# Enigmatisms/NeRF

Measured on AMD Instinct MI355X. Metric: rays/s (64+128 samples), 800x800, higher is better.
Workload: dtype bf16

## Files before the change

nerf_amd/csrc/sample_kernels.hip:

```cpp
#include "device_common.h"
#include "host_common.h"
#include "../../include/nerf_amd.h"
#include "launchers.h"

extern __shared__ __attribute__((aligned(16))) char smem[];

namespace {

constexpr int WAVES_PER_BLOCK = 4;

DEVINL int wave_in_block() { return (int)(threadIdx.x >> 6); }

constexpr int ENC_TILE = 64;
static inline size_t enc_lds_bytes(int L) { return (size_t)ENC_TILE * (6 * L + 6) * 4; }
template <bool IPE, class Moments>
DEVINL void encode_tile(float (*mom)[6], float* stage, int64_t base, int64_t total, int L, float* __restrict__ feat, Moments&& moments) {
    const int width = 6 * L, pairs_per = 3 * L;
    const int nsamp = (int)(total - base < ENC_TILE ? total - base : ENC_TILE);
    if ((int)threadIdx.x < nsamp) moments((int)threadIdx.x, base + threadIdx.x);
    __syncthreads();
    const int n_pairs = nsamp * pairs_per;
    for (int p = threadIdx.x; p < n_pairs; p += blockDim.x) {
        const int sl = p / pairs_per, rem = p - sl * pairs_per;
        const int l = rem / 3, c = rem - 3 * l;
// ... 305 lines not shown
            const int64_t k = cell / wp, r = cell - k * wp;
            const int64_t wr = r / ww;
            const int64_t row = y0 + wr, col = x0 + (r - wr * ww);
            const int64_t v = view_ids != nullptr ? view_ids[k] : k;
            float* q = ray_s[threadIdx.x];
            if (v >= 0 && v < V) {
                pixel_camera_ray((int)col, (int)row, cameras + v * NERF_AMD_CAMERA_ROW, poses + v * 12, q);
                const float* px = images + ((v * 3) * (int64_t)H + row) * W + col;
#pragma unroll
                for (int c = 0; c < 6; ++c) rays[n * 6 + c] = q[c];
#pragma unroll
                for (int c = 0; c < 3; ++c) rgb[n * 3 + c] = px[(int64_t)c * H * W];
                if (index != nullptr) index[n] = (v * H + row) * W + col;
            } else {
                const float nan = __builtin_nanf("");
#pragma unroll
                for (int c = 0; c < 6; ++c) { q[c] = nan; rays[n * 6 + c] = nan; }
#pragma unroll
                for (int c = 0; c < 3; ++c) rgb[n * 3 + c] = nan;
                if (index != nullptr) index[n] = -1;
            }
        }
        __syncthreads();
        if (lengths == nullptr) continue;
        sampler_samples(n0, N, C, seed, near, res, ray_s, lengths, pts);
    }
}

__global__ void length2pts_kernel(const float* __restrict__ rays, const float* __restrict__ z, int64_t N, int S,
                                  float* __restrict__ out) {
    const int64_t total = N * S * 6;
    for (int64_t i = blockIdx.x * (int64_t)blockDim.x + threadIdx.x; i < total; i += (int64_t)gridDim.x * blockDim.x) {
        const int64_t ns = i / 6;
        const int k = (int)(i - ns * 6);
        const int64_t n = ns / S;
        const float* r = rays + n * 6;
        out[i] = (k < 3) ? (r[k] + r[3 + k] * z[ns]) : r[k];
    }
}

__global__ __launch_bounds__(256) void sigma_to_weights_kernel(const float* __restrict__ sigma, const float* __restrict__ z,
                                                              const float* __restrict__ dirs, int64_t N, int S, int act,
                                                              float* __restrict__ w) {
    for (int64_t n = blockIdx.x * (int64_t)WAVES_PER_BLOCK + wave_in_block(); n < N; n += (int64_t)gridDim.x * WAVES_PER_BLOCK) {
        float nrm = 1.0f;
        const bool scale = dirs != nullptr;
        if (scale) nrm = norm3(dirs[n * 3], dirs[n * 3 + 1], dirs[n * 3 + 2]);
        const float* sg = sigma + n * S;
        const float* zz = z + n * S;
        float* wo = w + n * S;
        wave_sigma_to_weights(S, act, [&](int s) { return sg[s]; },
                              [&](int s) { return scale ? zz[s] * nrm : zz[s]; },
                              [&](int s, float wv, float) { wo[s] = wv; });
    }
}

DEVINL float max_blur_at(const float* w, int s, int S, float alpha) {
    const float c = w[s];
    const float front = (s == 0) ? c : fmaxf(w[s - 1], c);
    const float rear = (s == S - 1) ? c : fmaxf(c, w[s + 1]);
    return 0.5f * (front + rear) + alpha;
}
__global__ void max_blur_kernel(const float* __restrict__ w, int64_t N, int S, float alpha, float* __restrict__ out) {
    const int64_t total = N * S;
    for (int64_t i = blockIdx.x * (int64_t)blockDim.x + threadIdx.x; i < total; i += (int64_t)gridDim.x * blockDim.x) {
        const int s = (int)(i % S);
        out[i] = max_blur_at(w + (i - s), s, S, alpha);
    }
}

DEVINL void lds_wave_sync() {
    __builtin_amdgcn_fence(__ATOMIC_RELEASE, "workgroup");
    __builtin_amdgcn_wave_barrier();
    __builtin_amdgcn_fence(__ATOMIC_ACQUIRE, "workgroup");
}

#ifndef SORT_NB_DEF
#define SORT_NB_DEF 256
#define SORT_CAP_DEF 6
#endif
constexpr int SORT_NB = SORT_NB_DEF, SORT_CAP = SORT_CAP_DEF, SORT_PER_LANE = SORT_NB / 64;
constexpr int SORT_LDS_FLOATS = 2 * SORT_NB + SORT_NB * SORT_CAP / 2;

template <class UF>
DEVINL void wave_inverse_sample(const float* pw, const float* bins, int nw, float* cdf, float* samp, int* bel, int* sortbuf,
                                UF&& uf, int K, int sort, float* __restrict__ z_out,
                                int64_t* __restrict__ below_out, int64_t* __restrict__ above_out) {
    const int lane = lane_id();
    const int nb = nw + 1;
    float* part8 = reinterpret_cast<float*>(sortbuf);
    const int nv = nw >> 3;
    if (lane < 8) {
        const int n4 = nv >> 2;
        float a0 = 0.0f, a1 = 0.0f, a2 = 0.0f, a3 = 0.0f;
        for (int i = 0; i < n4; ++i) {
            a0 += pw[32 * i + lane] + 1e-5f;
            a1 += pw[32 * i + 8 + lane] + 1e-5f;
            a2 += pw[32 * i + 16 + lane] + 1e-5f;
            a3 += pw[32 * i + 24 + lane] + 1e-5f;
        }
        for (int v = 4 * n4; v < nv; ++v) a0 += pw[8 * v + lane] + 1e-5f;
        a0 += a1; a0 += a2; a0 += a3;
        part8[lane] = a0;
    }
    lds_wave_sync();
    float total = 0.0f;
    if (nv > 0) {
        for (int j = 8 * nv; j < nw; ++j) total += pw[j] + 1e-5f;
#pragma unroll
        for (int c = 0; c < 8; ++c) total += part8[c];
    } else {
        float a1 = 0.0f, a2 = 0.0f, a3 = 0.0f;
        if (nw >= 4) { total += pw[0] + 1e-5f; a1 += pw[1] + 1e-5f; a2 += pw[2] + 1e-5f; a3 += pw[3] + 1e-5f; }
        for (int j = nw & ~3; j < nw; ++j) total += pw[j] + 1e-5f;
        total += a1; total += a2; total += a3;
    }
    double carry = 0.0;
    if (lane == 0) cdf[0] = 0.0f;
    for (int base = 0; base < nw; base += 64) {
        const int j = base + lane;
        double p = 0.0;
        if (j < nw) p = (double)((pw[j] + 1e-5f) / total);
        const double incl = wave_incl_scan_add(p);
        if (j < nw) cdf[1 + j] = (float)(carry + incl);
        carry += wave_last(incl);
    }
    lds_wave_sync();
    const int halvings = 32 - __builtin_clz((unsigned)nb);
    for (int k0 = 0, i0 = 0; k0 < K; k0 += 192, i0 += 3) {
        float uu[3]; int lo[3], hi[3];
#pragma unroll
        for (int q = 0; q < 3; ++q) {
            const int k = k0 + 64 * q + lane;
            uu[q] = (k < K) ? uf(i0 + q, k) : 0.0f;
            lo[q] = 0; hi[q] = (k < K) ? nb : 0;
        }
        for (int it = 0; it < halvings; ++it) {
#pragma unroll
            for (int q = 0; q < 3; ++q) {
                const int mid = (lo[q] + hi[q]) >> 1;
                const bool open_ = lo[q] < hi[q];
                const float c = cdf[open_ ? mid : 0];
                if (open_) { if (c <= uu[q]) lo[q] = mid + 1; else hi[q] = mid; }
            }
        }
#pragma unroll
        for (int q = 0; q < 3; ++q) {
            const int k = k0 + 64 * q + lane;
            if (k >= K) continue;
            const int below = lo[q] - 1 > 0 ? lo[q] - 1 : 0;
            const int above = lo[q] < nb - 1 ? lo[q] : nb - 1;
            const float c0 = cdf[below], c1 = cdf[above];
            float denom = c1 - c0;
            if (denom < 1e-5f) denom = 1.0f;
            const float t = (uu[q] - c0) / denom;
            const float b0 = bins[below], b1 = bins[above];
            const float v = b0 + t * (b1 - b0);
            if (sort) { samp[k] = v; bel[k] = below; }
            else {
                z_out[k] = v;
                if (below_out) below_out[k] = below;
                if (above_out) above_out[k] = above;
            }
        }
    }
    if (!sort) return;
    lds_wave_sync();
    int* cnt = sortbuf;
    int* pre = sortbuf + SORT_NB;
    unsigned short* mem = reinterpret_cast<unsigned short*>(sortbuf + 2 * SORT_NB);
    for (int b = lane; b < SORT_NB; b += 64) cnt[b] = 0;
    lds_wave_sync();
    int overflow = 0, risky = -1;
    for (int j = lane; j + 1 < nb; j += 64) {
        const float b0 = bins[j], b1 = bins[j + 1];
        overflow |= (b1 < b0) ? 1 : 0;
        const bool exact = b0 >= 0.0f ? (b1 <= 2.0f * b0 || b0 == 0.0f) : (b1 <= 0.0f && b0 >= 2.0f * b1);
        if (!exact) risky = j;
    }
    if (__any(risky >= 0)) {
        risky = wave_max_i(risky);
        for (int k = lane; k < K; k += 64) {
            const int bl = bel[k];
            if (bl <= risky) overflow |= (samp[k] > bins[bl + 1]) ? 1 : 0;
        }
    }
    for (int k = lane, i = 0; k < K; k += 64, ++i) {
        int b = (int)(uf(i, k) * (float)SORT_NB);
        b = b < 0 ? 0 : (b > SORT_NB - 1 ? SORT_NB - 1 : b);
        const int pos = atomicAdd(&cnt[b], 1);
        if (pos < SORT_CAP) mem[b * SORT_CAP + pos] = (unsigned short)k; else overflow = 1;
    }
    lds_wave_sync();
    if (__any(overflow)) {
        for (int k = lane; k < K; k += 64) {
            const float v = samp[k];
            int rank = 0;
            for (int j = 0; j < K; ++j) {
                const float o = samp[j];
                rank += (o < v || (o == v && j < k)) ? 1 : 0;
            }
            z_out[rank] = v;
            if (below_out) below_out[rank] = bel[k];
        }
        return;
    }
    {
        int c[SORT_PER_LANE], tot = 0;
#pragma unroll
        for (int i = 0; i < SORT_PER_LANE; ++i) { c[i] = cnt[lane * SORT_PER_LANE + i]; tot += c[i]; }
        int run = wave_incl_scan_add(tot) - tot;
#pragma unroll
        for (int i = 0; i < SORT_PER_LANE; ++i) { pre[lane * SORT_PER_LANE + i] = run; run += c[i]; }
    }
    lds_wave_sync();
    for (int k0 = 0, i0 = 0; k0 < K; k0 += 192, i0 += 3) {
        float v[3]; int rank[3], cntb[3], bb[3];
#pragma unroll
        for (int q = 0; q < 3; ++q) {
            const int k = k0 + 64 * q + lane;
            const bool ok = k < K;
            int b = ok ? (int)(uf(i0 + q, k) * (float)SORT_NB) : 0;
            b = b < 0 ? 0 : (b > SORT_NB - 1 ? SORT_NB - 1 : b);
            bb[q] = b;
            v[q] = samp[ok ? k : 0];
            rank[q] = pre[b];
            cntb[q] = ok ? cnt[b] : 0;
        }
        int most = cntb[0] > cntb[1] ? cntb[0] : cntb[1];
        most = most > cntb[2] ? most : cntb[2];
        const int trips = wave_max_i(most);
        for (int p = 0; p < trips; ++p) {
#pragma unroll
            for (int q = 0; q < 3; ++q) {
                const int k = k0 + 64 * q + lane;
                const bool live = p < cntb[q];
                const int jx = mem[bb[q] * SORT_CAP + p];
                const float o = samp[live ? jx : 0];
                rank[q] += (live && (o < v[q] || (o == v[q] && jx < k))) ? 1 : 0;
            }
        }
#pragma unroll
        for (int q = 0; q < 3; ++q) {
            const int k = k0 + 64 * q + lane;
            if (k >= K) continue;
            z_out[rank[q]] = v[q];
            if (below_out) below_out[rank[q]] = bel[k];
        }
    }
}

template <class P> struct ResampleRowsAt { P pw, bins, cdf, samp, bel, sortbuf, zl, wraw, tail; };
typedef ResampleRowsAt<float*> ResampleRows;
template <class P> static inline __host__ __device__ ResampleRowsAt<P> resample_rows(P base, int C, int K) {
    ResampleRowsAt<P> r;
    r.pw = base; r.bins = r.pw + C; r.cdf = r.bins + C; r.samp = r.cdf + C; r.bel = r.samp + K; r.sortbuf = r.bel + K;
    r.zl = r.sortbuf + SORT_LDS_FLOATS; r.wraw = r.zl + C; r.tail = r.wraw + C;
    return r;
}
static inline __host__ __device__ size_t inv_lds_floats(int C, int K) { return resample_rows<size_t>(0, C, K).zl; }
static inline __host__ __device__ size_t rs_lds_floats(int C, int K) { return resample_rows<size_t>(0, C, K).tail; }
static inline __host__ __device__ size_t warped_lds_floats(int C, int K) { return rs_lds_floats(C, K) + (size_t)2 * K; }
static inline __host__ __device__ size_t rsw_lds_floats(int C, int K, bool warped) { return rs_lds_floats(C, K) + (size_t)(warped ? 2 : 1) * K; }
DEVINL ResampleRows wave_resample_rows(size_t wave_floats, int C, int K) {
    return resample_rows(reinterpret_cast<float*>(smem) + wave_in_block() * wave_floats, C, K);
}
template <class UF>
DEVINL void wave_inverse_sample(const ResampleRows& r, int nw, UF&& uf, int K, int sort, float* __restrict__ z_out, int64_t* __restrict__ below_out,
                                int64_t* __restrict__ above_out) {
    wave_inverse_sample(r.pw, r.bins, nw, r.cdf, r.samp, reinterpret_cast<int*>(r.bel), reinterpret_cast<int*>(r.sortbuf), uf, K, sort, z_out, below_out,
                        above_out);
}

DEVINL void wave_blur_pdf(const float* wraw, int C, float alpha, float* pw, float* w_prop) {
    for (int j = lane_id(); j < C; j += 64) {
        const float wb = max_blur_at(wraw, j, C, alpha);
        if (j >= 1 && j <= C - 2) pw[j - 1] = wb;
        if (w_prop) w_prop[j] = wb;
    }
}
DEVINL void wave_midpoints(const float* x, int C, float* bins) {
    for (int j = lane_id(); j < C - 1; j += 64) bins[j] = 0.5f * (x[j + 1] + x[j]);
}

__global__ __launch_bounds__(256) void inverse_sample_kernel(const float* __restrict__ w, const float* __restrict__ z,
                                                            const float* __restrict__ u, int64_t N, int C, int K, int sort,
                                                            int mode, float* __restrict__ z_out, int64_t* __restrict__ below,
                                                            int64_t* __restrict__ above) {
    const ResampleRows r = wave_resample_rows(inv_lds_floats(C, K), C, K);
    float* const pw = r.pw; float* const bins = r.bins;
    const int lane = lane_id();
    const int nw = mode == 0 ? C - 2 : C - 1;
    const int wstride = mode == 0 ? C : C - 1;
    for (int64_t n = blockIdx.x * (int64_t)WAVES_PER_BLOCK + wave_in_block(); n < N; n += (int64_t)gridDim.x * WAVES_PER_BLOCK) {
        lds_wave_sync();
        if (mode == 0) {
            for (int j = lane; j < nw; j += 64) pw[j] = w[n * wstride + 1 + j];
            wave_midpoints(z + n * C, C, bins);
        } else {
            for (int j = lane; j < nw; j += 64) pw[j] = w[n * wstride + j];
            for (int j = lane; j < nw + 1; j += 64) bins[j] = z[n * C + j];
        }
        lds_wave_sync();
        const float* un = u + n * K;
        wave_inverse_sample(r, nw, [&](int, int k) { return un[k]; }, K, sort, z_out + n * K, below ? below + n * K : nullptr,
                            above ? above + n * K : nullptr);
    }
}

struct ResampleArgs {
    const float* density; const float* z; const float* z_base; const float* u_strat; float z_jitter;
    const float* dirs; int dirs_stride; const float* u_inv; int64_t N; int C; int K; int softplus; float alpha;
    float* z_fine; int64_t* below; float* w_prop; float* z_coarse;
    uint64_t rng_seed; int64_t rng_ray_offset;
};

#ifndef RS_BLOCKS_PER_CU
#define RS_BLOCKS_PER_CU 5
#endif
__global__ __launch_bounds__(256) __attribute__((amdgpu_waves_per_eu(RS_BLOCKS_PER_CU, RS_BLOCKS_PER_CU))) void resample_kernel(ResampleArgs a) {
    const int C = a.C, K = a.K;
    const ResampleRows rows = wave_resample_rows(rs_lds_floats(C, K), C, K);
    float* const zl = rows.zl; float* const wraw = rows.wraw;
    const int lane = lane_id();
    struct RayIn { float dx, dy, dz, zv0, zv1, dens0, dens1, u0, u1, u2; };
    const bool fits = C <= 128 && K <= 192;
    auto load_in = [&](int64_t n) -> RayIn {
        RayIn r;
        const float* dd = a.dirs + n * a.dirs_stride;
        r.dx = dd[0]; r.dy = dd[1]; r.dz = dd[2];
        Philox4 blk = {{0u, 0u, 0u, 0u}};
        const bool draw = !a.u_inv || (!a.z && !a.u_strat);
        if (draw) blk = philox_ray_block(a.rng_seed, n + a.rng_ray_offset, lane);
        auto depth_of = [&](int j, bool first) {
            if (a.z) return a.z[n * C + j];
            const float uu = a.u_strat ? a.u_strat[n * C + j] : (first ? u01_from_bits(blk.w[0]) : philox_u_strat(a.rng_seed, n + a.rng_ray_offset, j));
            return a.z_base[j] + uu * a.z_jitter;
        };
        r.zv0 = r.zv1 = r.dens0 = r.dens1 = 0.0f;
        if (lane < C) { r.zv0 = depth_of(lane, true); r.dens0 = a.density[n * C + lane]; }
        if (lane + 64 < C) { r.zv1 = depth_of(lane + 64, false); r.dens1 = a.density[n * C + lane + 64]; }
        if (a.u_inv) {
            const float* un = a.u_inv + n * K;
            r.u0 = (lane < K) ? un[lane] : 0.0f;
            r.u1 = (lane + 64 < K) ? un[lane + 64] : 0.0f;
            r.u2 = (lane + 128 < K) ? un[lane + 128] : 0.0f;
        } else {
            r.u0 = u01_from_bits(blk.w[1]); r.u1 = u01_from_bits(blk.w[2]); r.u2 = u01_from_bits(blk.w[3]);
        }
        return r;
    };
    const int64_t stride = (int64_t)gridDim.x * WAVES_PER_BLOCK;
    int64_t n = blockIdx.x * (int64_t)WAVES_PER_BLOCK + wave_in_block();
    if (n >= a.N) return;
    RayIn cur = {};
    if (fits) cur = load_in(n);
    for (; n < a.N; n += stride) {
        RayIn nxt = cur;
        if (fits && n + stride < a.N) nxt = load_in(n + stride);
        lds_wave_sync();
        float nrm;
        if (fits) {
            nrm = norm3(cur.dx, cur.dy, cur.dz);
            if (lane < C) { zl[lane] = cur.zv0; if (a.z_coarse) a.z_coarse[n * C + lane] = cur.zv0; }
            if (lane + 64 < C) { zl[lane + 64] = cur.zv1; if (a.z_coarse) a.z_coarse[n * C + lane + 64] = cur.zv1; }
        } else {
            const float* dd = a.dirs + n * a.dirs_stride;
            nrm = norm3(dd[0], dd[1], dd[2]);
            for (int j = lane; j < C; j += 64) {
                const float zv = a.z ? a.z[n * C + j]
                                     : (a.z_base[j] + (a.u_strat ? a.u_strat[n * C + j] : philox_u_strat(a.rng_seed, n + a.rng_ray_offset, j)) * a.z_jitter);
                zl[j] = zv;
                if (a.z_coarse) a.z_coarse[n * C + j] = zv;
            }
        }
        lds_wave_sync();
        const float* sg = a.density + n * C;
        const int soft = a.softplus;
        const float dens0 = cur.dens0, dens1 = cur.dens1, cu0 = cur.u0, cu1 = cur.u1, cu2 = cur.u2;
        wave_sigma_to_weights(C, NERF_AMD_ACT_RELU,
                              [=](int s) { const float d = fits ? ((s >> 6) ? dens1 : dens0) : sg[s]; return soft ? softplus_f(d) : d; },
                              [=](int s) { return zl[s] * nrm; },
                              [=](int s, float wv, float) { wraw[s] = wv; });
        lds_wave_sync();
        wave_blur_pdf(wraw, C, a.alpha, rows.pw, a.w_prop ? a.w_prop + n * C : nullptr);
        wave_midpoints(zl, C, rows.bins);
        lds_wave_sync();
        const float* un = a.u_inv ? a.u_inv + n * K : nullptr;
        const uint64_t seed = a.rng_seed; const int64_t nn = n + a.rng_ray_offset;
        wave_inverse_sample(rows, C - 2,
                            [=](int i, int k) {
                                if (fits) return i == 0 ? cu0 : (i == 1 ? cu1 : cu2);
                                if (un) return un[k];
                                return philox_u_inv(seed, nn, k);
                            },
                            K, 1, a.z_fine + n * K, a.below ? a.below + n * K : nullptr, nullptr);
        cur = nxt;
    }
}

struct WarpConsts { float near, far, gn, gf; };
DEVINL float warp_s_to_z(float s, const WarpConsts& c) {
    const float sb = fminf(fmaxf(s, 0.0f), 1.0f);
    return 1.0f / ((1.0f - sb) * c.gn + sb * c.gf);
}
DEVINL float warp_z_to_s(float z, const WarpConsts& c) {
    const float zb = fminf(fmaxf(z, c.near), c.far);
    return (1.0f / zb - c.gn) / (c.gf - c.gn);
}

__global__ void warp_depths_kernel(const float* __restrict__ in, const float* __restrict__ rays, int64_t N, int S, int inverse, WarpConsts c,
                                   float* __restrict__ out, float* __restrict__ pts) {
    const int64_t total = N * S;
    for (int64_t i = blockIdx.x * (int64_t)blockDim.x + threadIdx.x; i < total; i += (int64_t)gridDim.x * blockDim.x) {
        const float zv = inverse ? warp_z_to_s(in[i], c) : warp_s_to_z(in[i], c);
        out[i] = zv;
        if (pts) point_on_ray(rays + (i / S) * 6, zv, pts + i * 3);
    }
}

__global__ void warped_stratified_kernel(const float* __restrict__ rays, const float* __restrict__ u, int64_t N, int C, float res, uint64_t seed,
                                         int64_t ray_offset, WarpConsts c, float* __restrict__ s_out, float* __restrict__ z_out,
                                         float* __restrict__ pts) {
    const int64_t total = N * C;
    for (int64_t i = blockIdx.x * (int64_t)blockDim.x + threadIdx.x; i < total; i += (int64_t)gridDim.x * blockDim.x) {
        const int64_t n = i / C;
        const int j = (int)(i - n * C);
        const float uu = u ? u[i] : philox_u_strat(seed, n + ray_offset, j);
        const float sv = (float)j * res + uu * res;
        const float zv = warp_s_to_z(sv, c);
        s_out[i] = sv;
        z_out[i] = zv;
        if (pts) point_on_ray(rays + n * 6, zv, pts + i * 3);
    }
}

DEVINL void wave_unwarp_samples(const float* sf, int K, const WarpConsts& c, float* s_fine, float* z_fine) {
    for (int k = lane_id(); k < K; k += 64) {
        const float sv = sf[k];
        if (s_fine) s_fine[k] = sv;
        z_fine[k] = warp_s_to_z(sv, c);
    }
}

struct WarpedResampleArgs {
    const float* density; const float* s_c; const float* dirs; int dirs_stride; const float* u_inv; int64_t N; int C; int K; int softplus;
    float alpha; WarpConsts c; float* z_fine; float* s_fine; int64_t* below; float* w_prop; uint64_t rng_seed; int64_t rng_ray_offset;
};

__global__ __launch_bounds__(256) void warped_resample_kernel(WarpedResampleArgs a) {
    const int C = a.C, K = a.K;
    const ResampleRows rows = wave_resample_rows(warped_lds_floats(C, K), C, K);
    float* const zl = rows.zl; float* const wraw = rows.wraw;
    float* const sf = rows.tail; float* const uu = sf + K;
    const int lane = lane_id();
    const WarpConsts c = a.c;
    for (int64_t n = blockIdx.x * (int64_t)WAVES_PER_BLOCK + wave_in_block(); n < a.N; n += (int64_t)gridDim.x * WAVES_PER_BLOCK) {
        lds_wave_sync();
        const float* dd = a.dirs + n * a.dirs_stride;
        const float nrm = norm3(dd[0], dd[1], dd[2]);
        const float* sc = a.s_c + n * C;
        for (int j = lane; j < C; j += 64) zl[j] = warp_s_to_z(sc[j], c);
        const int64_t nn = n + a.rng_ray_offset;
        for (int k = lane; k < K; k += 64) uu[k] = a.u_inv ? a.u_inv[n * K + k] : philox_u_inv(a.rng_seed, nn, k);
        lds_wave_sync();
        const float* sg = a.density + n * C;
        const int soft = a.softplus;
        wave_sigma_to_weights(C, NERF_AMD_ACT_RELU,
                              [=](int s) { const float d = sg[s]; return soft ? softplus_f(d) : d; },
                              [=](int s) { return zl[s] * nrm; },
                              [=](int s, float wv, float) { wraw[s] = wv; });
        lds_wave_sync();
        wave_blur_pdf(wraw, C, a.alpha, rows.pw, a.w_prop ? a.w_prop + n * C : nullptr);
        wave_midpoints(sc, C, rows.bins);
        lds_wave_sync();
        wave_inverse_sample(rows, C - 2, [=](int, int k) { return uu[k]; }, K, 1, sf, a.below ? a.below + n * K : nullptr, nullptr);
        lds_wave_sync();
        wave_unwarp_samples(sf, K, c, a.s_fine ? a.s_fine + n * K : nullptr, a.z_fine + n * K);
// ... 1287 lines not shown
    }
}
int nk::sk_philox_normal(float* out, int64_t M, uint64_t seed, const uint64_t* seed_dev, float std, int64_t sample_offset, hipStream_t st) {
    if (M == 0) return 0;
    hipLaunchKernelGGL(philox_normal_kernel, dim3(blocks_for(M * 16, 256)), dim3(256), 0, st, out, M, seed, seed_dev, std, sample_offset);
    return (int)hipGetLastError();
}
__global__ void advance_seed_kernel(uint64_t* __restrict__ seed_dev) {
    uint64_t x = seed_dev[0] + 0x9E3779B97F4A7C15ull;
    x = (x ^ (x >> 30)) * 0xBF58476D1CE4E5B9ull;
    x = (x ^ (x >> 27)) * 0x94D049BB133111EBull;
    seed_dev[0] = x ^ (x >> 31);
}
int nk::sk_philox_uniforms(float* out, int64_t N, int K, uint64_t seed, const uint64_t* seed_dev, int64_t ray_offset, int strat, hipStream_t st) {
    if (N * K == 0) return 0;
    hipLaunchKernelGGL(philox_uniforms_kernel, dim3(blocks_for(N * K, 256)), dim3(256), 0, st, out, N, K, seed, seed_dev, ray_offset, strat);
    return (int)hipGetLastError();
}
int nk::sk_advance_seed(uint64_t* seed_dev, hipStream_t st) {
    hipLaunchKernelGGL(advance_seed_kernel, dim3(1), dim3(1), 0, st, seed_dev);
    return (int)hipGetLastError();
}
int nk::sk_generate_rays(const float* pose, int H, int W, float fx, float fy, int64_t first, int64_t count, float* rays,
                     hipStream_t st) {
    Cam c; c.H = H; c.W = W; c.fx = fx; c.fy = fy;
    for (int i = 0; i < 12; ++i) c.pose[i] = pose[i];
    if (count == 0) return 0;
    hipLaunchKernelGGL(raygen_kernel, dim3(blocks_for(count, 256)), dim3(256), 0, st, c, first, count, rays);
    return (int)hipGetLastError();
}
int nk::sk_generate_rays_camera(const float* pose, int H, int W, const float* camera, int64_t first, int64_t count, float* rays, hipStream_t st) {
    Cam c; c.H = H; c.W = W; c.fx = camera[0]; c.fy = camera[1];
    for (int i = 0; i < 12; ++i) c.pose[i] = pose[i];
    CameraRow row;
    for (int i = 0; i < NERF_AMD_CAMERA_ROW; ++i) row.v[i] = camera[i];
    if (count == 0) return 0;
    hipLaunchKernelGGL(raygen_camera_kernel, dim3(blocks_for(count, 256)), dim3(256), 0, st, row, c, first, count, rays);
    return (int)hipGetLastError();
}
int nk::sk_pixel_rays(const float* pose, float fx, float fy, const int64_t* coords, int64_t N, float* rays, hipStream_t st) {
    Cam c; c.H = 0; c.W = 0; c.fx = fx; c.fy = fy;
    for (int i = 0; i < 12; ++i) c.pose[i] = pose[i];
    if (N == 0) return 0;
    hipLaunchKernelGGL(pixel_rays_kernel, dim3(blocks_for(N, 256)), dim3(256), 0, st, c, coords, N, rays);
    return (int)hipGetLastError();
}
int nk::sk_stratified_points(const float* rays, const float* z_base, const float* u, float jitter, int64_t N, int S, float* z_out,
                         float* pts, hipStream_t st) {
    if (N * S == 0) return 0;
    hipLaunchKernelGGL(stratified_points_kernel, dim3(blocks_for(N * S, 256)), dim3(256), 0, st, rays, z_base, u, jitter, N, S, z_out, pts);
    return (int)hipGetLastError();
}
int nk::sk_length2pts(const float* rays, const float* z, int64_t N, int S, float* out, hipStream_t st) {
    if (N * S == 0) return 0;
    hipLaunchKernelGGL(length2pts_kernel, dim3(blocks_for(N * S * 6, 256)), dim3(256), 0, st, rays, z, N, S, out);
    return (int)hipGetLastError();
}
int nk::sk_sigma_to_weights(const float* sigma, const float* z, const float* dirs, int64_t N, int S, int act, float* w, hipStream_t st) {
    if (N * S == 0) return 0;
    hipLaunchKernelGGL(sigma_to_weights_kernel, dim3(blocks_for(N, WAVES_PER_BLOCK)), dim3(256), 0, st, sigma, z, dirs, N, S, act, w);
    return (int)hipGetLastError();
}
int nk::sk_max_blur(const float* w, int64_t N, int S, float alpha, float* out, hipStream_t st) {
    if (N * S == 0) return 0;
    hipLaunchKernelGGL(max_blur_kernel, dim3(blocks_for(N * S, 256)), dim3(256), 0, st, w, N, S, alpha, out);
    return (int)hipGetLastError();
}
int nk::sk_inverse_sample(const float* w, const float* z, const float* u, int64_t N, int C, int K, int sort, int mode, float* z_out,
                      int64_t* below, int64_t* above, hipStream_t st) {
    if (N == 0) return 0;
    hipLaunchKernelGGL(inverse_sample_kernel, dim3(blocks_for(N, WAVES_PER_BLOCK)), dim3(256), sk_inverse_sample_lds_bytes(C, K), st, w, z, u, N, C, K, sort, mode,
                       z_out, below, above);
    return (int)hipGetLastError();
}
int nk::sk_resample(const float* density, const float* z, const float* z_base, const float* u_strat, float z_jitter,
                const float* dirs, int dirs_stride, const float* u_inv, int64_t N, int C, int K, int softplus, float alpha,
                uint64_t rng_seed, int64_t rng_ray_offset, float* z_fine, int64_t* below, float* w_prop, float* z_coarse, hipStream_t st) {
    if (N == 0) return 0;
    ResampleArgs a{density, z, z_base, u_strat, z_jitter, dirs, dirs_stride, u_inv, N, C, K, softplus, alpha, z_fine, below, w_prop, z_coarse,
                   rng_seed, rng_ray_offset};
    int64_t blocks = (N + WAVES_PER_BLOCK - 1) / WAVES_PER_BLOCK;
    const int64_t resident = (int64_t)nerf_host::cu_count() * RS_BLOCKS_PER_CU;
    if (blocks > resident) blocks = resident;
    hipLaunchKernelGGL(resample_kernel, dim3((unsigned)blocks), dim3(256), sk_resample_lds_bytes(C, K), st, a);
    return (int)hipGetLastError();
}
int nk::sk_warp_depths(const float* in, const float* rays, int64_t N, int S, int inverse, float near, float far, float gn, float gf, float* out, float* pts,
                   hipStream_t st) {
    if (N * S == 0) return 0;
    hipLaunchKernelGGL(warp_depths_kernel, dim3(blocks_for(N * S, 256)), dim3(256), 0, st, in, rays, N, S, inverse, WarpConsts{near, far, gn, gf}, out, pts);
    return (int)hipGetLastError();
}
int nk::sk_warped_stratified(const float* rays, const float* u, int64_t N, int C, uint64_t seed, int64_t ray_offset, float near, float far, float gn, float gf,
                         float* s_out, float* z_out, float* pts, hipStream_t st) {
    if (N * C == 0) return 0;
    hipLaunchKernelGGL(warped_stratified_kernel, dim3(blocks_for(N * C, 256)), dim3(256), 0, st, rays, u, N, C, 1.0f / (float)C, seed, ray_offset,
                       WarpConsts{near, far, gn, gf}, s_out, z_out, pts);
    return (int)hipGetLastError();
}
int nk::sk_warped_resample(const float* density, const float* s_c, const float* dirs, int dirs_stride, const float* u_inv, int64_t N, int C, int K, int softplus,
                       float alpha, float near, float far, float gn, float gf, uint64_t rng_seed, int64_t rng_ray_offset, float* z_fine, float* s_fine,
                       int64_t* below, float* w_prop, hipStream_t st) {
    if (N == 0) return 0;
    WarpedResampleArgs a{density, s_c, dirs, dirs_stride, u_inv, N, C, K, softplus, alpha, WarpConsts{near, far, gn, gf}, z_fine, s_fine, below, w_prop,
                         rng_seed, rng_ray_offset};
    hipLaunchKernelGGL(warped_resample_kernel, dim3(blocks_for(N, WAVES_PER_BLOCK)), dim3(256), sk_warped_resample_lds_bytes(C, K), st, a);
    return (int)hipGetLastError();
}
int nk::sk_resample_window(const float* density, const float* z, const float* dirs, int dirs_stride, int64_t N, int C, int K, int u_col0, float alpha,
                       uint64_t rng_seed, int64_t rng_ray_offset, float* z_fine, hipStream_t st) {
    if (N == 0) return 0;
    ResampleWindowArgs a{density, z, dirs, dirs_stride, N, C, K, u_col0, alpha, WarpConsts{}, z_fine, nullptr, rng_seed, rng_ray_offset};
    hipLaunchKernelGGL(resample_window_kernel<false>, dim3(blocks_for(N, WAVES_PER_BLOCK)), dim3(256), sk_resample_window_lds_bytes(C, K, 0), st, a);
    return (int)hipGetLastError();
}
int nk::sk_warped_resample_window(const float* density, const float* s_c, const float* dirs, int dirs_stride, int64_t N, int C, int K, int u_col0, float alpha,
                              float near, float far, float gn, float gf, uint64_t rng_seed, int64_t rng_ray_offset, float* z_fine, float* s_fine, hipStream_t st) {
    if (N == 0) return 0;
    ResampleWindowArgs a{density, s_c, dirs, dirs_stride, N, C, K, u_col0, alpha, WarpConsts{near, far, gn, gf}, z_fine, s_fine, rng_seed, rng_ray_offset};
    hipLaunchKernelGGL(resample_window_kernel<true>, dim3(blocks_for(N, WAVES_PER_BLOCK)), dim3(256), sk_resample_window_lds_bytes(C, K, 1), st, a);
    return (int)hipGetLastError();
}
int nk::sk_composite(const float* rgbo, const float* z, int z_stride, const float* dirs, int dirs_stride, int64_t N, int S, int flags,
                 int act, float sigma_shift, float near, float far, const float* normal, const float* cam_dir, float* rgb, float* weights,
                 float* depth, float* normal_img, hipStream_t st) {
    if (N == 0) return 0;
    CompositeArgs a{rgbo, z, z_stride, dirs, dirs_stride, N, S, flags, act, sigma_shift, near, far, normal, cam_dir, rgb, weights, depth, normal_img};
    hipLaunchKernelGGL(composite_kernel, dim3(blocks_for(N, WAVES_PER_BLOCK)), dim3(256), 0, st, a);
    return (int)hipGetLastError();
}
int nk::sk_composite_rows(const float* rgbo, const int32_t* row_of_ray, const float* z, int z_stride, const float* dirs, int dirs_stride, int64_t N, int S, int flags,
                      int act, float sigma_shift, float near, float far, const float* normal, const float* cam_dir, float* rgb, float* weights, float* depth,
                      float* normal_img, hipStream_t st) {
    if (N == 0) return 0;
    CompositeArgs a{rgbo, z, z_stride, dirs, dirs_stride, N, S, flags, act, sigma_shift, near, far, normal, cam_dir, rgb, weights, depth, normal_img};
    hipLaunchKernelGGL(composite_rows_kernel, dim3(blocks_for(N, WAVES_PER_BLOCK)), dim3(256), 0, st, a, row_of_ray);
    return (int)hipGetLastError();
}
size_t nk::sk_ray_alive_workspace_bytes(int64_t N) {
    const size_t n = (size_t)N, tiles = (n + ALIVE_TILE - 1) / ALIVE_TILE;
    return ((n + 255) & ~(size_t)255) + ((tiles * 4 + 255) & ~(size_t)255) + 256;
}
int nk::sk_ray_alive(const float* density, const float* z, int z_stride, const float* dirs, int dirs_stride, int64_t N, int C, double d_min, int32_t* row_of_ray,
                 int64_t* ray_of_row, int64_t* count_dev, void* workspace, hipStream_t st) {
    if (N == 0) return (int)hipMemsetAsync(count_dev, 0, 8, st);
    uint8_t* flags = reinterpret_cast<uint8_t*>((reinterpret_cast<uintptr_t>(workspace) + 255) & ~(uintptr_t)255);
    int* tiles = reinterpret_cast<int*>(flags + (((size_t)N + 255) & ~(size_t)255));
    const int64_t n_tiles = (N + ALIVE_TILE - 1) / ALIVE_TILE;
    RayAliveArgs a{density, z, z_stride, dirs, dirs_stride, N, C, d_min, flags};
    hipLaunchKernelGGL(ray_alive_kernel, dim3(blocks_for(N, WAVES_PER_BLOCK)), dim3(256), 0, st, a);
    hipLaunchKernelGGL(alive_count_kernel, dim3((unsigned)n_tiles), dim3(256), 0, st, flags, N, tiles);
    hipLaunchKernelGGL(alive_offsets_kernel, dim3(1), dim3(256), 0, st, tiles, n_tiles, count_dev);
    hipLaunchKernelGGL(alive_tables_kernel, dim3((unsigned)n_tiles), dim3(256), 0, st, flags, N, tiles, row_of_ray, ray_of_row);
    return (int)hipGetLastError();
}
int nk::sk_gather_rows(const float* src, int64_t src_stride, const int64_t* ray_of_row, int64_t n_rows, int cols, float* dst, hipStream_t st) {
    if (n_rows * cols == 0) return 0;
    hipLaunchKernelGGL(gather_rows_kernel, dim3(blocks_for(n_rows * cols, 256)), dim3(256), 0, st, src, src_stride, ray_of_row, n_rows, cols, dst);
    return (int)hipGetLastError();
}
int nk::sk_ray_depth_stats(const float* w, const float* z, int z_stride, int closed, const float* dirs, int dirs_stride, int64_t N, int S, int mul_norm,
                           const float* quantiles, int n_quantiles, float near, float far, float* opacity, float* depth_q, hipStream_t st) {
    if (N == 0 || (!opacity && !(depth_q && n_quantiles))) return 0;
    DepthStatsArgs a{w, z, z_stride, closed ? 1 : 0, dirs, dirs_stride, N, S, mul_norm ? 1 : 0, {}, depth_q ? n_quantiles : 0, near, far, opacity, depth_q};
    for (int j = 0; j < a.nq; ++j) a.q[j] = quantiles[j];
    hipLaunchKernelGGL(ray_depth_stats_kernel, dim3(blocks_for(N, WAVES_PER_BLOCK)), dim3(256), 0, st, a);
    return (int)hipGetLastError();
// ... 151 lines not shown
```

Measured before the change: 10.03 million.

## Handle small tail of inverse-CDF draws with wave ballots and add render resample kernel

```diff
diff --git a/nerf_amd/csrc/sample_kernels.hip b/nerf_amd/csrc/sample_kernels.hip
--- a/nerf_amd/csrc/sample_kernels.hip
+++ b/nerf_amd/csrc/sample_kernels.hip
@@ -411,7 +411,16 @@
 constexpr int SORT_NB = SORT_NB_DEF, SORT_CAP = SORT_CAP_DEF, SORT_PER_LANE = SORT_NB / 64;
 constexpr int SORT_LDS_FLOATS = 2 * SORT_NB + SORT_NB * SORT_CAP / 2;
 
-template <class UF>
+#ifndef TAIL_MAX_DEF
+#define TAIL_MAX_DEF 4
+#endif
+constexpr int TAIL_MAX = TAIL_MAX_DEF;
+static_assert(TAIL_MAX >= 1 && TAIL_MAX < 64, "the render shape K = 129 has a tail of one draw");
+template <int NQ, bool TAILS, class UF>
+DEVINL void wave_draw_and_sort(const float* bins, int nb, const float* cdf, float* samp, int* bel, int* sortbuf, UF&& uf, int K, int Km, int sort,
+                               float* __restrict__ z_out, int64_t* __restrict__ below_out, int64_t* __restrict__ above_out);
+
+template <bool TAILS = true, class UF>
 DEVINL void wave_inverse_sample(const float* pw, const float* bins, int nw, float* cdf, float* samp, int* bel, int* sortbuf,
                                 UF&& uf, int K, int sort, float* __restrict__ z_out,
                                 int64_t* __restrict__ below_out, int64_t* __restrict__ above_out) {
@@ -444,6 +453,10 @@
         for (int j = nw & ~3; j < nw; ++j) total += pw[j] + 1e-5f;
         total += a1; total += a2; total += a3;
     }
+    const int tail = K & 63;
+    const bool tail_shape = TAILS && K >= 64 && K < 192 && tail >= 1 && tail <= TAIL_MAX;
+    bool unordered = false;
+    float last_c = 0.0f;
     double carry = 0.0;
     if (lane == 0) cdf[0] = 0.0f;
     for (int base = 0; base < nw; base += 64) {
@@ -451,22 +464,46 @@
         double p = 0.0;
         if (j < nw) p = (double)((pw[j] + 1e-5f) / total);
         const double incl = wave_incl_scan_add(p);
-        if (j < nw) cdf[1 + j] = (float)(carry + incl);
+        const float cv = (float)(carry + incl);
+        if (j < nw) cdf[1 + j] = cv;
+        if (tail_shape) {
+            const float lower = dpp_move<DPP_WAVE_SHR1, 0xF>(last_c, cv);
+            unordered |= j < nw && !(lower <= cv);
+            last_c = __builtin_bit_cast(float, __builtin_amdgcn_readlane(__builtin_bit_cast(int, cv), 63));
+        }
         carry += wave_last(incl);
     }
     lds_wave_sync();
+    const int r = (tail_shape && !__any(unordered)) ? tail : 0;
+    const int Km = K - r;
+    if (!TAILS || Km > 128) wave_draw_and_sort<3, TAILS>(bins, nb, cdf, samp, bel, sortbuf, uf, K, Km, sort, z_out, below_out, above_out);
+    else if (Km <= 64) wave_draw_and_sort<1, TAILS>(bins, nb, cdf, samp, bel, sortbuf, uf, K, Km, sort, z_out, below_out, above_out);
+    else wave_draw_and_sort<2, TAILS>(bins, nb, cdf, samp, bel, sortbuf, uf, K, Km, sort, z_out, below_out, above_out);
+}
+
+DEVINL float lane_value(float v, int l) { return __builtin_bit_cast(float, __builtin_amdgcn_readlane(__builtin_bit_cast(int, v), l)); }
+DEVINL int sort_bucket(float u) {
+    const int b = (int)(u * (float)SORT_NB);
+    return b < 0 ? 0 : (b > SORT_NB - 1 ? SORT_NB - 1 : b);
+}
+
+template <int NQ, bool TAILS, class UF>
+DEVINL void wave_draw_and_sort(const float* bins, int nb, const float* cdf, float* samp, int* bel, int* sortbuf, UF&& uf, int K, int Km, int sort,
+                               float* __restrict__ z_out, int64_t* __restrict__ below_out, int64_t* __restrict__ above_out) {
+    const int lane = lane_id();
+    const int r = (TAILS && NQ < 3) ? K - Km : 0;
     const int halvings = 32 - __builtin_clz((unsigned)nb);
-    for (int k0 = 0, i0 = 0; k0 < K; k0 += 192, i0 += 3) {
-        float uu[3]; int lo[3], hi[3];
-#pragma unroll
-        for (int q = 0; q < 3; ++q) {
+    for (int k0 = 0, i0 = 0; k0 < Km; k0 += 64 * NQ, i0 += NQ) {
+        float uu[NQ]; int lo[NQ], hi[NQ];
+#pragma unroll
+        for (int q = 0; q < NQ; ++q) {
             const int k = k0 + 64 * q + lane;
-            uu[q] = (k < K) ? uf(i0 + q, k) : 0.0f;
-            lo[q] = 0; hi[q] = (k < K) ? nb : 0;
+            uu[q] = (k < Km) ? uf(i0 + q, k) : 0.0f;
+            lo[q] = 0; hi[q] = (k < Km) ? nb : 0;
         }
         for (int it = 0; it < halvings; ++it) {
 #pragma unroll
-            for (int q = 0; q < 3; ++q) {
+            for (int q = 0; q < NQ; ++q) {
                 const int mid = (lo[q] + hi[q]) >> 1;
                 const bool open_ = lo[q] < hi[q];
                 const float c = cdf[open_ ? mid : 0];
@@ -474,9 +511,9 @@
             }
         }
 #pragma unroll
-        for (int q = 0; q < 3; ++q) {
+        for (int q = 0; q < NQ; ++q) {
             const int k = k0 + 64 * q + lane;
-            if (k >= K) continue;
+            if (k >= Km) continue;
             const int below = lo[q] - 1 > 0 ? lo[q] - 1 : 0;
             const int above = lo[q] < nb - 1 ? lo[q] : nb - 1;
             const float c0 = cdf[below], c1 = cdf[above];
@@ -493,6 +530,36 @@
             }
         }
     }
+    auto tail_uniform = [&]() { return lane < r ? uf(Km >> 6, Km + lane) : 0.0f; };
+    if (r > 0) {
+        const float ut = tail_uniform();
+        for (int t = 0; t < r; ++t) {
+            const float u = lane_value(ut, t);
+            int lo = 0;
+            for (int base = 0; base < nb; base += 64) {
+                const int j = base + lane;
+                const float c = cdf[j < nb ? j : 0];
+                lo += __popcll(__ballot(j < nb && c <= u));
+            }
+            const int k = Km + t;
+            const int below = lo - 1 > 0 ? lo - 1 : 0;
+            const int above = lo < nb - 1 ? lo : nb - 1;
+            const float c0 = cdf[below], c1 = cdf[above];
+            float denom = c1 - c0;
+            if (denom < 1e-5f) denom = 1.0f;
+            const float tt = (u - c0) / denom;
+            const float b0 = bins[below], b1 = bins[above];
+            const float v = b0 + tt * (b1 - b0);
+            if (lane == 0) {
+                if (sort) { samp[k] = v; bel[k] = below; }
+                else {
+                    z_out[k] = v;
+                    if (below_out) below_out[k] = below;
+                    if (above_out) above_out[k] = above;
+                }
+            }
+        }
+    }
     if (!sort) return;
     lds_wave_sync();
     int* cnt = sortbuf;
@@ -514,13 +581,19 @@
             if (bl <= risky) overflow |= (samp[k] > bins[bl + 1]) ? 1 : 0;
         }
     }
-    for (int k = lane, i = 0; k < K; k += 64, ++i) {
-        int b = (int)(uf(i, k) * (float)SORT_NB);
-        b = b < 0 ? 0 : (b > SORT_NB - 1 ? SORT_NB - 1 : b);
+    for (int k = lane, i = 0; k < Km; k += 64, ++i) {
+        const int b = sort_bucket(uf(i, k));
         const int pos = atomicAdd(&cnt[b], 1);
         if (pos < SORT_CAP) mem[b * SORT_CAP + pos] = (unsigned short)k; else overflow = 1;
     }
     lds_wave_sync();
+    if (r > 0) {
+        const int bt = sort_bucket(tail_uniform());
+        for (int t = 0; t < r; ++t) {
+            const int b = __builtin_amdgcn_readlane(bt, t);
+            if (cnt[b] + __popcll(__ballot(lane < r && bt == b)) > SORT_CAP) overflow = 1;
+        }
+    }
     if (__any(overflow)) {
         for (int k = lane; k < K; k += 64) {
             const float v = samp[k];
@@ -543,25 +616,26 @@
         for (int i = 0; i < SORT_PER_LANE; ++i) { pre[lane * SORT_PER_LANE + i] = run; run += c[i]; }
     }
     lds_wave_sync();
-    for (int k0 = 0, i0 = 0; k0 < K; k0 += 192, i0 += 3) {
-        float v[3]; int rank[3], cntb[3], bb[3];
-#pragma unroll
-        for (int q = 0; q < 3; ++q) {
+    int rt = 0;
+    for (int k0 = 0, i0 = 0; k0 < Km; k0 += 64 * NQ, i0 += NQ) {
+        float v[NQ]; int rank[NQ], cntb[NQ], bb[NQ];
+#pragma unroll
+        for (int q = 0; q < NQ; ++q) {
             const int k = k0 + 64 * q + lane;
-            const bool ok = k < K;
-            int b = ok ? (int)(uf(i0 + q, k) * (float)SORT_NB) : 0;
-            b = b < 0 ? 0 : (b > SORT_NB - 1 ? SORT_NB - 1 : b);
+            const bool ok = k < Km;
+            const int b = ok ? sort_bucket(uf(i0 + q, k)) : 0;
             bb[q] = b;
             v[q] = samp[ok ? k : 0];
             rank[q] = pre[b];
             cntb[q] = ok ? cnt[b] : 0;
         }
-        int most = cntb[0] > cntb[1] ? cntb[0] : cntb[1];
-        most = most > cntb[2] ? most : cntb[2];
+        int most = cntb[0];
+#pragma unroll
+        for (int q = 1; q < NQ; ++q) most = most > cntb[q] ? most : cntb[q];
         const int trips = wave_max_i(most);
         for (int p = 0; p < trips; ++p) {
 #pragma unroll
-            for (int q = 0; q < 3; ++q) {
+            for (int q = 0; q < NQ; ++q) {
                 const int k = k0 + 64 * q + lane;
                 const bool live = p < cntb[q];
                 const int jx = mem[bb[q] * SORT_CAP + p];
@@ -569,12 +643,41 @@
                 rank[q] += (live && (o < v[q] || (o == v[q] && jx < k))) ? 1 : 0;
             }
         }
-#pragma unroll
-        for (int q = 0; q < 3; ++q) {
+        const int bt = r > 0 ? sort_bucket(tail_uniform()) : 0;
+        for (int t = 0; t < r; ++t) {
+            const int bT = __builtin_amdgcn_readlane(bt, t);
+            const float vT = samp[Km + t];
+            int front = 0;
+#pragma unroll
+            for (int q = 0; q < NQ; ++q) {
+                const bool ok = k0 + 64 * q + lane < Km;
+                const bool same = bb[q] == bT;
+                front += __popcll(__ballot(ok && (bb[q] < bT || (same && (v[q] < vT || v[q] == vT)))));
+                rank[q] += (bT < bb[q] || (same && vT < v[q])) ? 1 : 0;
+            }
+            if (lane == t) rt += front;
+        }
+#pragma unroll
+        for (int q = 0; q < NQ; ++q) {
             const int k = k0 + 64 * q + lane;
-            if (k >= K) continue;
+            if (k >= Km) continue;
             z_out[rank[q]] = v[q];
             if (below_out) below_out[rank[q]] = bel[k];
+        }
+    }
+    if (r > 0) {
+        const int bt = sort_bucket(tail_uniform());
+        const float vt = samp[lane < r ? Km + lane : 0];
+        const int belt = bel[lane < r ? Km + lane : 0];
+        int rank = rt;
+        for (int t = 0; t < r; ++t) {
+            const int bT = __builtin_amdgcn_readlane(bt, t);
+            const float vT = lane_value(vt, t);
+            rank += (bT < bt || (bT == bt && (vT < vt || (vT == vt && t < lane)))) ? 1 : 0;
+        }
+        if (lane < r) {
+            z_out[rank] = vt;
+            if (below_out) below_out[rank] = belt;
         }
     }
 }
@@ -594,10 +697,10 @@
 DEVINL ResampleRows wave_resample_rows(size_t wave_floats, int C, int K) {
     return resample_rows(reinterpret_cast<float*>(smem) + wave_in_block() * wave_floats, C, K);
 }
-template <class UF>
+template <bool TAILS = true, class UF>
 DEVINL void wave_inverse_sample(const ResampleRows& r, int nw, UF&& uf, int K, int sort, float* __restrict__ z_out, int64_t* __restrict__ below_out,
                                 int64_t* __restrict__ above_out) {
-    wave_inverse_sample(r.pw, r.bins, nw, r.cdf, r.samp, reinterpret_cast<int*>(r.bel), reinterpret_cast<int*>(r.sortbuf), uf, K, sort, z_out, below_out,
+    wave_inverse_sample<TAILS>(r.pw, r.bins, nw, r.cdf, r.samp, reinterpret_cast<int*>(r.bel), reinterpret_cast<int*>(r.sortbuf), uf, K, sort, z_out, below_out,
                         above_out);
 }
 
@@ -717,12 +820,80 @@
         lds_wave_sync();
         const float* un = a.u_inv ? a.u_inv + n * K : nullptr;
         const uint64_t seed = a.rng_seed; const int64_t nn = n + a.rng_ray_offset;
-        wave_inverse_sample(rows, C - 2,
+        wave_inverse_sample<false>(rows, C - 2,
                             [=](int i, int k) {
                                 if (fits) return i == 0 ? cu0 : (i == 1 ? cu1 : cu2);
                                 if (un) return un[k];
                                 return philox_u_inv(seed, nn, k);
                             },
+                            K, 1, a.z_fine + n * K, a.below ? a.below + n * K : nullptr, nullptr);
+        cur = nxt;
+    }
+}
+
+template <bool PHILOX, bool SOFTPLUS>
+__global__ __launch_bounds__(256) __attribute__((amdgpu_waves_per_eu(RS_BLOCKS_PER_CU, RS_BLOCKS_PER_CU))) void resample_render_kernel(ResampleArgs a) {
+    const int C = a.C, K = a.K;
+    __builtin_assume(K <= 192);
+    const ResampleRows rows = wave_resample_rows(rs_lds_floats(C, K), C, K);
+    float* const zl = rows.zl; float* const wraw = rows.wraw;
+    const int lane = lane_id();
+    struct RayIn { float dx, dy, dz, zv, dens, u0, u1, u2; };
+    auto load_in = [&](int64_t n) -> RayIn {
+        RayIn r;
+        const float* dd = a.dirs + n * a.dirs_stride;
+        r.dx = dd[0]; r.dy = dd[1]; r.dz = dd[2];
+        r.zv = r.dens = 0.0f;
+        if (PHILOX) {
+            const Philox4 blk = philox_ray_block(a.rng_seed, n + a.rng_ray_offset, lane);
+            if (lane < C) r.zv = a.z_base[lane] + u01_from_bits(blk.w[0]) * a.z_jitter;
+            r.u0 = u01_from_bits(blk.w[1]); r.u1 = u01_from_bits(blk.w[2]); r.u2 = u01_from_bits(blk.w[3]);
+        } else {
+            if (lane < C) r.zv = a.z_base[lane] + a.u_strat[n * C + lane] * a.z_jitter;
+            const float* un = a.u_inv + n * K;
+            r.u0 = (lane < K) ? un[lane] : 0.0f;
+            r.u1 = (lane + 64 < K) ? un[lane + 64] : 0.0f;
+            r.u2 = (lane + 128 < K) ? un[lane + 128] : 0.0f;
+        }
+        if (lane < C) r.dens = a.density[n * C + lane];
+        return r;
+    };
+    const int64_t stride = (int64_t)gridDim.x * WAVES_PER_BLOCK;
+    int64_t n = blockIdx.x * (int64_t)WAVES_PER_BLOCK + wave_in_block();
+    if (n >= a.N) return;
+    const bool ok = lane < C;
+    RayIn cur = load_in(n);
+    for (; n < a.N; n += stride) {
+        RayIn nxt = cur;
+        if (n + stride < a.N) nxt = load_in(n + stride);
+        lds_wave_sync();
+        const float nrm = norm3(cur.dx, cur.dy, cur.dz);
+        if (ok) { zl[lane] = cur.zv; if (a.z_coarse) a.z_coarse[n * C + lane] = cur.zv; }
+        lds_wave_sync();
+        {
+            float w = 0.0f;
+            double p = 1.0;
+            if (ok) {
+                const float z0 = zl[lane] * nrm;
+                const float delta = (lane + 1 < C) ? (zl[lane + 1] * nrm - z0) : 1e10f;
+                const float m = expf(-density_act(SOFTPLUS ? softplus_f(cur.dens) : cur.dens, NERF_AMD_ACT_RELU) * delta);
+                w = 1.0f - m;
+                p = (double)(m + 1e-10f);
+            }
+            const double excl = wave_shift_up1(wave_incl_scan_mul(p), 1.0);
+            const float T = (float)excl;
+            if (ok) wraw[lane] = w * T;
+        }
+        lds_wave_sync();
+        if (ok) {
+            const float wb = max_blur_at(wraw, lane, C, a.alpha);
+            if (lane >= 1 && lane <= C - 2) rows.pw[lane - 1] = wb;
+            if (a.w_prop) a.w_prop[n * C + lane] = wb;
+            if (lane < C - 1) rows.bins[lane] = 0.5f * (zl[lane + 1] + zl[lane]);
+        }
+        lds_wave_sync();
+        const float cu0 = cur.u0, cu1 = cur.u1, cu2 = cur.u2;
+        wave_inverse_sample(rows, C - 2, [=](int i, int) { return i == 0 ? cu0 : (i == 1 ? cu1 : cu2); },
                             K, 1, a.z_fine + n * K, a.below ? a.below + n * K : nullptr, nullptr);
         cur = nxt;
     }
@@ -2176,7 +2347,12 @@
     int64_t blocks = (N + WAVES_PER_BLOCK - 1) / WAVES_PER_BLOCK;
     const int64_t resident = (int64_t)nerf_host::cu_count() * RS_BLOCKS_PER_CU;
     if (blocks > resident) blocks = resident;
-    hipLaunchKernelGGL(resample_kernel, dim3((unsigned)blocks), dim3(256), sk_resample_lds_bytes(C, K), st, a);
+    const bool philox = !u_strat && !u_inv;
+    void (*kernel)(ResampleArgs) = resample_kernel;
+    if (C <= 64 && K <= 192 && !z && (philox || (u_strat && u_inv)))
+        kernel = philox ? (softplus ? resample_render_kernel<true, true> : resample_render_kernel<true, false>)
+                        : (softplus ? resample_render_kernel<false, true> : resample_render_kernel<false, false>);
+    hipLaunchKernelGGL(kernel, dim3((unsigned)blocks), dim3(256), sk_resample_lds_bytes(C, K), st, a);
     return (int)hipGetLastError();
 }
 int nk::sk_warp_depths(const float* in, const float* rays, int64_t N, int S, int inverse, float near, float far, float gn, float gf, float* out, float* pts,
```

Result: no change. 10.07 million, median of 6 (+0.4%).
